# fjetter/distributed

Hardware: AMD Instinct MI355X
Metric: task placements/sec at 1M tasks x 1,024 workers; % of HBM roofline (higher is better)
Workload: dtype int64+f64

## Files before the change

distributed_amd/csrc/dgp_stream.h:

```cpp

#include "dgp_svcmsg.h"

#ifndef DGP_ST_NS
#define DGP_ST_NS st
#endif

#ifndef DGP_STREAM_SHARED_DEFINED
#define DGP_STREAM_SHARED_DEFINED
#define DGP_ST_PRIMARY 1
namespace dgp {
constexpr size_t ST_LDS_BYTES = 22608;
__shared__ __attribute__((aligned(16))) char st_lds_raw[ST_LDS_BYTES];
extern __shared__ __attribute__((aligned(16))) char st_smem[];
}
#else
#undef DGP_ST_PRIMARY
#define DGP_ST_PRIMARY 0
#endif

namespace dgp {
namespace DGP_ST_NS {

__constant__ Dev c_dev;

#ifndef DGP_PHASE_PROBES
#define DGP_PHASE_PROBES 0
#endif
#ifndef DGP_EXE_PRIO
#define DGP_EXE_PRIO 1
#endif
#ifndef DGP_EXE_SLEEP
#define DGP_EXE_SLEEP 1
#endif
#ifndef DGP_EXE_PF
#define DGP_EXE_PF 1
#endif
#ifndef DGP_PROF_GLOBAL
#define DGP_PROF_GLOBAL 0
#endif
#ifndef DGP_REG_PROBES
#define DGP_REG_PROBES 0
#endif
#ifndef DGP_BULK_RESTR
#define DGP_BULK_RESTR 1
#endif
#ifndef DGP_RUN_PAR
#define DGP_RUN_PAR 1
#endif
#ifndef DGP_RB
#define DGP_RB 8
#endif
#ifndef DGP_SCTA
#define DGP_SCTA 1024
#endif
constexpr int SCTA = DGP_SCTA;
#ifndef DGP_WIN
#define DGP_WIN 32
#endif
constexpr int WIN = DGP_WIN;
using SMask = unsigned long long;
static_assert(WIN >= 32 && WIN <= 64, "DGP_WIN must be in [32, 64]");
#ifndef DGP_WAITC
#define DGP_WAITC 1
#endif
constexpr bool WAITC = DGP_WAITC != 0;
constexpr int WAITC_AHEAD = 32;
static_assert(!WAITC || WIN == 32, "DGP_WAITC keeps the candidate-only registrations in the masks' high half");
__host__ __device__ constexpr unsigned long long slot_bits(int s) {
  return WAITC ? ((1ull << s) | (1ull << (s + 32))) : (1ull << s);
}
#ifndef DGP_RS
#define DGP_RS 128
#endif
constexpr int RS = DGP_RS;
constexpr int NE = 64;
#ifndef DGP_DR
#define DGP_DR 512
#endif
constexpr int DR = DGP_DR;
constexpr int PLC = 64;
constexpr int KT_MAX = 24;
constexpr int KX_MAX = 8;
constexpr int RC_MAX = 8;
constexpr int PD = 8;
constexpr int PX = 32;
constexpr int TMAX = 32;
constexpr int NLW = 12;
constexpr int NXW = 52;
constexpr int PG = 64;
constexpr int BIG = 1 << 24;
constexpr int T_CAND = 0x8000;
constexpr int T_W = 0x7fff;
constexpr uint32_t NL_OVF = 0xffffffffu;
static_assert(NLW == SNLW && NXW == SNXW && NL_OVF == SNL_OVF, "dgp_device.h's one-lane needs_what ops use this layout");
constexpr int N_ROLE = 5;
constexpr int E_HDR = 7;
static_assert((DR & (DR - 1)) == 0 && DR >= 64 && DR >= WIN, "DGP_DR must be a power of two >= 64");
static_assert((RS & (RS - 1)) == 0 && RS >= WIN && RS <= DR, "DGP_RS must be a power of two in [WIN, DR]");

enum : uint32_t { F_GLOBAL = 1, F_SELFREL = 2, F_EXACT = 4, F_TOUCHALL = 8, F_BADTOUCH = 16, F_SIMPLE = 32, F_RUNM = 64 };
enum : int { K_COMPLETE = 1, K_PLACE = 2, K_COMPLETE_LR = 3 };
enum : int { SERR_NONE = 0, SERR_PREFIX = 11, SERR_WATCHDOG = 12, SERR_QUEUE = 13, SERR_NEEDS = 14,
             SERR_REC = 15, SERR_CAND = 16, SERR_STAGE = 17, SERR_RANGE = 18, SERR_INV = 19 };

#if DGP_ST_PRIMARY
struct Pos {
  long long seq, bld, pre, reg;
  long long rec_len, walk;
  long long runid_upto;
  long long round_end;
  long long round_start_saved;
  long long prev_placed;
};

struct SRec {
  int32_t w;
  int16_t p;
  int8_t kind;
  int8_t pad;
  int32_t nproc;
  int32_t task;
  int64_t dnet;
  double occ;
  double dur;
};
#else
using st::Pos;
using st::SRec;
#endif

struct SCtl {
  int stop, error, err_task;
  int inv_ok;
  int q_anon;
  int q_prefix;
  int capmax;
  int global_pending;
// ... 339 lines not shown
      sl[PD - 1] = 0u;
      ord -= 1u << 24;
    }
  }
  const bool lj = lane_id() == j;
  d.c.x = lj ? sl[0] : d.c.x;
  d.c.y = lj ? sl[1] : d.c.y;
  d.c.z = lj ? sl[2] : d.c.z;
  d.c.w = lj ? sl[3] : d.c.w;
  d.c1.x = lj ? sl[4] : d.c1.x;
  d.c1.y = lj ? sl[5] : d.c1.y;
  d.c1.z = lj ? sl[6] : d.c1.z;
  d.c1.w = lj ? sl[7] : d.c1.w;
  d.ord = lj ? ord : d.ord;
  return ok;
}

using DTab = const __attribute__((address_space(3))) double*;

__device__ __forceinline__ double resolve_dur(const Dev& D, double d, int p) {
  return d < 0 ? (D.pmaxexec[p] > 0 ? 2 * D.pmaxexec[p] : D.unknown_duration) : d;
}

__device__ __forceinline__ double occ_dict(const WDict& d, int64_t netocc, DTab dt, const Dev& D) {
  const uint32_t n = wd_n(d.ord);
  double res = 0.0;
#pragma unroll
  for (int i = 0; i < PD; i++) {
    if (!ballot((uint32_t)i < n)) break;
    const uint32_t v = wd_slot(d, i);
    const int p = (int)(v >> 24) & (PX - 1);
    const double dv = dt[p];
    const double term = resolve_dur(D, dv, p) * (double)(v & 0xffffffu);
    if ((uint32_t)i < n) res += term;
  }
  return res + (double)netocc / (double)D.bandwidth;
}

__device__ __forceinline__ double occ_dict_r(const WDict& d, double net_bw, DTab dt, const Dev& D) {
  const uint32_t n = wd_n(d.ord);
  double res = 0.0;
  {
    const uint32_t v0 = d.c.x, v1 = d.c.y;
    const double dv0 = dt[(v0 >> 24) & (PX - 1)], dv1 = dt[(v1 >> 24) & (PX - 1)];
    const double t0 = (dv0 < 0 ? D.unknown_duration : dv0) * (double)(v0 & 0xffffffu);
    const double t1 = (dv1 < 0 ? D.unknown_duration : dv1) * (double)(v1 & 0xffffffu);
    if (n > 0u) res += t0;
    if (n > 1u) res += t1;
  }
#pragma unroll
  for (int i = 2; i < PD; i++) {
    if (!ballot((uint32_t)i < n)) break;
    const uint32_t v = wd_slot(d, i);
    const double dv = dt[(v >> 24) & (PX - 1)];
    const double term = (dv < 0 ? D.unknown_duration : dv) * (double)(v & 0xffffffu);
    if ((uint32_t)i < n) res += term;
  }
  return res + net_bw;
}
__device__ __forceinline__ double net_bw_of(int64_t netocc, const Dev& D) {
  return (double)netocc / (double)D.bandwidth;
}

template <bool LW>
__device__ __forceinline__ WDict dict_load(const WPtr<LW>& P, int c) {
  using U4 = typename WPtr<LW>::template P<const Q4>;
  WDict d;
  d.c = ld4(ascast<U4>(P.pcnt + (size_t)c * PD));
  d.c1 = ld4(ascast<U4>(P.pcnt + (size_t)c * PD + 4));
  d.ord = P.plen[c];
  return d;
}

template <bool LW>
__device__ __forceinline__ double occ_of(const WPtr<LW>& P, const Dev& D, int c, DTab dt) {
  return occ_dict(dict_load<LW>(P, c), P.netocc[c], dt, D);
}


__device__ __attribute__((always_inline)) void serr(SCtl& S, int code, int task) {
  if (atomicCAS(&S.error, 0, code) == 0) S.err_task = task;
  vstore(&S.stop, 1);
}


constexpr unsigned long long WATCHDOG = 1600000000ull;
__device__ __forceinline__ unsigned long long rclk() { return __builtin_amdgcn_s_memrealtime(); }
__device__ __forceinline__ bool stalled_for(unsigned long long since, unsigned long long now) {
  return now - since > WATCHDOG;
}

__device__ __forceinline__ int64_t nbv(const Dev& D, int64_t v) { return v >= 0 ? v : D.default_data_size; }
__device__ __forceinline__ bool restr_has(const Dev& D, int x, int w) {
  const RRow rr = restr_row(D, x);
  int64_t lo = rr.r0, hi = rr.r1;
  while (lo < hi) {
    const int64_t mid = (lo + hi) >> 1;
    if (rr.idx[mid] < w) lo = mid + 1;
    else hi = mid;
  }
  return lo < rr.r1 && rr.idx[lo] == w;
}

struct WState {
  int n;
  int pf;
  long long cnt;
  double netocc;
  double wd;
  long long n_idle, n_sat;
};
static_assert(PG == 64 && PX <= 64, "one lane per global dict entry / per prefix");

__device__ __forceinline__ int64_t rl_i64(int64_t v, int l) { return mk64(rlu(lo32(v), l), rlu(hi32(v), l)); }
__device__ __forceinline__ double rl_f64(double v, int l) { return mkd(rlu(dlo(v), l), rlu(dhi(v), l)); }

__device__ __forceinline__ void ws_load(const SCtl& S, WState& g) {
  const int lane = lane_id();
  g.n = S.g_plen;
  g.pf = S.g_pfx[lane];
  g.cnt = S.g_pcnt[lane];
  g.netocc = S.g_netocc;
  g.wd = S.wdur[lane & (PX - 1)];
  g.n_idle = S.n_idle;
  g.n_sat = S.n_sat;
}
__device__ __forceinline__ void ws_store(SCtl& S, const WState& g) {
  const int lane = lane_id();
  if (lane == 0) {
    S.g_plen = g.n;
    S.g_netocc = g.netocc;
    S.n_idle = g.n_idle;
    S.n_sat = g.n_sat;
  }
  S.g_pfx[lane] = g.pf;
  S.g_pcnt[lane] = g.cnt;
  if (lane < PX) S.wdur[lane] = g.wd;
}
__device__ __forceinline__ bool gdict_add(WState& g, int p, int delta) {
  const int lane = lane_id();
  const unsigned long long m = ballot(lane < g.n && g.pf == p);
  if (delta > 0) {
    if (m) {
      if (lane == __builtin_ctzll(m)) g.cnt++;
      return true;
    }
    if (g.n >= PG) return false;
    if (lane == g.n) {
      g.pf = p;
      g.cnt = 1;
    }
    g.n++;
    return true;
  }
  if (!m) return true;
  const int at = __builtin_ctzll(m);
  const long long v = rl_i64(g.cnt, at) - 1;
  if (v > 0) {
    if (lane == at) g.cnt = v;
    return true;
  }
  const int pn = __shfl_down(g.pf, 1);
  const long long cn = __shfl_down(g.cnt, 1);
  if (lane >= at) {
    g.pf = pn;
    g.cnt = cn;
// ... 1239 lines not shown
  if (m) {
    const int ml = __builtin_ctzll(m);
    const uint32_t v = rlu(nl, ml) - 1;
    const bool gone = (v & 0xffu) == 0;
    if (lane == ml) nl = gone ? 0u : v;
    if (gone && lane == NLW - 1) nl -= 0x100u;
    return gone ? nb : 0;
  }
  const int ext = (int)(ctl >> 8) - line_used(nl);
  if (ext > 0) {
    uint32_t* X = D.gw_needs_ext + (size_t)c * NXW;
    const uint32_t xe = lane < NXW ? __hip_atomic_load(X + lane, __ATOMIC_RELAXED, __HIP_MEMORY_SCOPE_AGENT) : 0u;
    const unsigned long long mx = ballot(lane < NXW && xe != 0 && (xe >> 8) == (uint32_t)d);
    if (mx) {
      const int ml = __builtin_ctzll(mx);
      const uint32_t v = rlu(xe, ml) - 1;
      const bool gone = (v & 0xffu) == 0;
      if (lane == ml) __hip_atomic_store(X + ml, gone ? 0u : v, __ATOMIC_RELAXED, __HIP_MEMORY_SCOPE_AGENT);
      if (gone && lane == NLW - 1) nl -= 0x100u;
      __threadfence_block();
      return gone ? nb : 0;
    }
  }
  if (D.evf & EVF_MULTI) return 0;
  serr(S, SERR_NEEDS, d);
  return 0;
}

__device__ __attribute__((always_inline)) int64_t needs_inc(const Dev& D, SCtl& S, int c, uint32_t& nl, int d, int64_t nb, int except) {
  const int lane = lane_id();
  const uint32_t ctl = rlu(nl, NLW - 1);
  if (ctl == NL_OVF) return st_needed_elsewhere(D, d, c, except) ? 0 : nb;
  const unsigned long long m = ballot(lane < NLW - 1 && nl != 0 && (nl >> 8) == (uint32_t)d);
  if (m) {
    const int ml = __builtin_ctzll(m);
    if ((rlu(nl, ml) & 0xffu) == 0xffu) {
      serr(S, SERR_NEEDS, d);
      return 0;
    }
    if (lane == ml) nl += 1;
    return 0;
  }
  const int used = line_used(nl);
  const int ext = (int)(ctl >> 8) - used;
  uint32_t* X = D.gw_needs_ext + (size_t)c * NXW;
  uint32_t xe = 0;
  if (ext > 0) {
    xe = lane < NXW ? __hip_atomic_load(X + lane, __ATOMIC_RELAXED, __HIP_MEMORY_SCOPE_AGENT) : 0u;
    const unsigned long long mx = ballot(lane < NXW && xe != 0 && (xe >> 8) == (uint32_t)d);
    if (mx) {
      const int ml = __builtin_ctzll(mx);
      if ((rlu(xe, ml) & 0xffu) == 0xffu) {
        serr(S, SERR_NEEDS, d);
        return 0;
      }
      if (lane == ml) __hip_atomic_store(X + ml, xe + 1, __ATOMIC_RELAXED, __HIP_MEMORY_SCOPE_AGENT);
      __threadfence_block();
      return 0;
    }
  }
  const unsigned long long em = ballot(lane < NLW - 1 && nl == 0);
  if (em) {
    if (lane == __builtin_ctzll(em)) nl = ((uint32_t)d << 8) | 1u;
    if (lane == NLW - 1) nl += 0x100u;
    return nb;
  }
  if (ext < NXW) {
    const unsigned long long ex = ballot(lane < NXW && xe == 0);
    const int ml = __builtin_ctzll(ex);
    if (lane == ml) __hip_atomic_store(X + ml, ((uint32_t)d << 8) | 1u, __ATOMIC_RELAXED, __HIP_MEMORY_SCOPE_AGENT);
    if (lane == NLW - 1) nl = nl + 0x100u;
    __threadfence_block();
    return nb;
  }
  if (lane == NLW - 1) nl = NL_OVF;
  return nb;
}

__device__ __forceinline__ unsigned long long lm_eq(unsigned a, unsigned b) { return __builtin_amdgcn_uicmp(a, b, 32); }
__device__ __forceinline__ unsigned long long lm_ne(unsigned a, unsigned b) { return __builtin_amdgcn_uicmp(a, b, 33); }
__device__ __forceinline__ bool lm_has(unsigned long long m) { return (m >> lane_id()) & 1ull; }
constexpr unsigned long long NL_LINE = (1ull << (NLW - 1)) - 1;

__device__ __forceinline__ bool needs_dec_all(const uint4& E, int L0, int k, int c, uint32_t& nl, int64_t& freed) {
  const uint32_t ctl = rlu(nl, NLW - 1);
  const unsigned long long used = lm_ne(nl, 0u) & NL_LINE;
  if (ctl == NL_OVF || (int)(ctl >> 8) != __builtin_popcountll(used)) return false;
  const uint32_t key = nl >> 8;
  const unsigned long long one = lm_eq(nl & 0xffu, 1u) & used;
  unsigned long long hit = 0;
  int64_t fr = 0;
  int ngone = 0;
  for (int i = 0; i < k; i++) {
    if (rl((int)E.y, L0 + i) == c) continue;
    const unsigned long long m = lm_eq(key, rlu(E.x, L0 + i)) & used;
    if (!m) return false;
    hit |= m;
    if (m & one) {
      fr += mk64(rlu(E.z, L0 + i), rlu(E.w, L0 + i));
      ngone++;
    }
  }
  if (hit) nl = lm_has(hit & one) ? 0u : (lm_has(hit) ? nl - 1u : nl);
  if (ngone) nl = lane_id() == NLW - 1 ? nl - ((uint32_t)ngone << 8) : nl;
  freed = fr;
  return true;
}

__device__ __forceinline__ bool needs_inc_all(const uint4& E, int L0, int k, int c, uint32_t& nl, int64_t& added) {
  const uint32_t ctl = rlu(nl, NLW - 1);
  const unsigned long long used = lm_ne(nl, 0u) & NL_LINE;
  if (ctl == NL_OVF || (int)(ctl >> 8) != __builtin_popcountll(used)) return false;
  const uint32_t key = nl >> 8;
  const unsigned long long full = lm_eq(nl & 0xffu, 0xffu) & used;
  unsigned long long freem = ~used & NL_LINE;
  unsigned long long hit = 0;
  uint32_t nn = nl;
  int64_t ad = 0;
  int nins = 0;
  for (int i = 0; i < k; i++) {
    if (rl((int)E.y, L0 + i) == c) continue;
    const uint32_t d = rlu(E.x, L0 + i);
    const unsigned long long m = lm_eq(key, d) & used;
    if (m) {
      if (m & full) return false;
      hit |= m;
    } else {
      if (!freem) return false;
      const int l = __builtin_ctzll(freem);
      freem &= freem - 1;
      nn = lane_id() == l ? (d << 8) | 1u : nn;
      ad += mk64(rlu(E.z, L0 + i), rlu(E.w, L0 + i));
      nins++;
    }
  }
  if (hit) nn = lm_has(hit) ? nn + 1u : nn;
  if (nins) nn = lane_id() == NLW - 1 ? nn + ((uint32_t)nins << 8) : nn;
  nl = nn;
  added = ad;
  return true;
}

__device__ __attribute__((always_inline)) void needs_reset(const Dev& D, int c, uint32_t& nl) {
  const int lane = lane_id();
  const uint32_t ctl = rlu(nl, NLW - 1);
  if (ctl == NL_OVF || (ctl >> 8) != 0) {
    if (lane < NXW) __hip_atomic_store(D.gw_needs_ext + (size_t)c * NXW + lane, 0u, __ATOMIC_RELAXED, __HIP_MEMORY_SCOPE_AGENT);
    __threadfence_block();
  }
  if (lane < NLW) nl = 0;
}

struct Out {
  int nrec, npl;
  size_t st0;
  __device__ void rec(const Dev& D, int kind, int w, int p, int64_t dnet, double occ, int np, int task, double dur) {
    if (lane_id() == 0 && nrec < PLC) {
      SRec rc;
      rc.w = w;
      rc.p = (int16_t)p;
      rc.kind = (int8_t)kind;
      rc.pad = 0;
      rc.nproc = np;
      rc.task = task;
      rc.dnet = dnet;
      rc.occ = occ;
      rc.dur = dur;
      D.srec[st0 + nrec] = rc;
    }
    nrec++;
  }
  __device__ void place(const Dev& D, int task, int w, int64_t comm, double start, int64_t wsnb, int route) {
    if (lane_id() == 0 && npl < PLC) {
      D.s2_task[st0 + npl] = task;
      D.s2_worker[st0 + npl] = w;
      D.s2_comm[st0 + npl] = comm;
      D.s2_start[st0 + npl] = start;
      D.s2_wsnb[st0 + npl] = wsnb;
      D.s2_route[st0 + npl] = (int8_t)route;
    }
    npl++;
  }
};

template <bool LW>
__device__ __forceinline__ bool dict_update(const WPtr<LW>& P, int c, int p, int delta, WDict& d) {
  using U4 = typename WPtr<LW>::template P<Q4>;
  d = dict_load<LW>(P, c);
  const bool ok = dict_add(d, p, delta);
  if (lane_id() == 0) {
    st4(ascast<U4>(P.pcnt + (size_t)c * PD), d.c);
    st4(ascast<U4>(P.pcnt + (size_t)c * PD + 4), d.c1);
    P.plen[c] = d.ord;
  }
  return ok;
}

__device__ __forceinline__ int release_succ(SLds& L, SMask old, int from = -1) {
  const SMask succ = WAITC ? (old & 0xffffffffull) : old;
  if (!succ) return -1;
  int bs = __builtin_ctzll(succ);
  long long best = vload(&L.sid[bs]);
  for (SMask m = succ & (succ - 1); m; m &= m - 1) {
    const int b = __builtin_ctzll(m);
    const long long v = vload(&L.sid[b]);
    if (v < best) {
      best = v;
      bs = b;
    }
  }
  if (WAITC && ((old >> 32) >> bs) & 1ull) {
    const int pc = __hip_atomic_fetch_add(&L.predc[bs], -1, __ATOMIC_RELAXED, __HIP_MEMORY_SCOPE_WORKGROUP);
    if (TR3 && pc == 1) {
      const Dev& D = c_dev;
      TR(L.sid[bs], 20);
      if (from >= 0) trace_at(D, L.sid[bs], 21, (unsigned long long)L.sid[from]);
    }
    return -1;
// ... 1 lines not shown
  if (atomicSub(&L.pred[bs], 1) == 1) {
    atomicOr(&L.c.ready, 1ull << bs);
    if (TRL) {
      const Dev& D = c_dev;
      TR(L.sid[bs], 1);
      if (TR3 && from >= 0) trace_at(D, L.sid[bs], 19, (unsigned long long)L.sid[from]);
    }
    return bs;
  }
  return -1;
}
template <bool LW>
__device__ __forceinline__ int release_worker(SLds& L, const WPtr<LW>& P, int s, int c) {
  const SMask bit = slot_bits(s);
  return release_succ(L, __hip_atomic_fetch_and(&P.mask[c], ~bit, __ATOMIC_RELAXED, __HIP_MEMORY_SCOPE_WORKGROUP) & ~bit,
                      DGP_TRACE ? s : -1);
}

template <bool LW>
__device__ __attribute__((always_inline)) void release_slot(const Dev& D, SLds& L, const WPtr<LW>& P, int s, bool all) {
  const int lane = lane_id();
  const SMask bit = slot_bits(s);
  auto rel = [&](int c) {
    release_succ(L, __hip_atomic_fetch_and(&P.mask[c], ~bit, __ATOMIC_RELAXED, __HIP_MEMORY_SCOPE_WORKGROUP) & ~bit,
                 DGP_TRACE ? s : -1);
  };
  if (all) {
    for (int c = lane; c < D.W; c += 64) rel(c);
  } else {
    const int nt = L.ntouch[s];
    if (lane < nt) rel((int)L.touch[s][lane] & T_W);
  }
}

template <class O>
__device__ __attribute__((always_inline)) void finish_slot(const Dev& D, SLds& L, int s, long long r, const O& o, int npops, bool direct) {
  const int lane = lane_id();
  const int q = (int)(r & (RS - 1));
  if (lane == 0) {
    RMeta me;
    me.npl = o.npl;
    me.nrec = (uint8_t)(direct ? 0 : o.nrec);
    me.npops = (uint8_t)npops;
    me.direct = direct ? 1 : 0;
    me.pad = 0;
    L.rmeta[q] = me;
  }
  __threadfence_block();
  if (lane == 0) {
    vstore(&L.rdone[q], r + 1);
    atomicOr(&L.c.freem, 1ull << s);
  }
  if (DGP_TRACE && lane == 0) TR(r, 5);
}

__device__ __forceinline__ unsigned wmin_u32(unsigned v) {
  v = min(v, (unsigned)__builtin_amdgcn_update_dpp((int)v, (int)v, 0xb1, 0xf, 0xf, false));
  v = min(v, (unsigned)__builtin_amdgcn_update_dpp((int)v, (int)v, 0x4e, 0xf, 0xf, false));
  v = min(v, (unsigned)__builtin_amdgcn_update_dpp((int)v, (int)v, 0x141, 0xf, 0xf, false));
  v = min(v, (unsigned)__builtin_amdgcn_update_dpp((int)v, (int)v, 0x140, 0xf, 0xf, false));
  return min(min(rlu(v, 0), rlu(v, 16)), min(rlu(v, 32), rlu(v, 48)));
}

struct Key {
  double start;
  int64_t nb;
  int w;
  int64_t comm;
};
__device__ __forceinline__ bool key_less(const Key& a, const Key& b) {
  if (a.start != b.start) return a.start < b.start;
  if (a.nb != b.nb) return a.nb < b.nb;
  return a.w < b.w;
}

__device__ __forceinline__ uint64_t start_key(double x) {
  const uint64_t b = x == 0.0 ? 0ull : (uint64_t)__double_as_longlong(x);
  return (b >> 63) ? ~b : (b | (1ull << 63));
}
__device__ __forceinline__ uint64_t rl64(uint64_t v, int l) {
  return ((uint64_t)rlu((unsigned)(v >> 32), l) << 32) | rlu((unsigned)v, l);
}

__device__ __forceinline__ DTab stim_durations(const Dev& D, SLds& L, const uint4& E, long long r) {
  const int lane = lane_id();
  const auto t = (__attribute__((address_space(3))) double*)(double*)L.dur[threadIdx.x >> 6];
  if (D.P <= PD) {
    if (lane >= 3 && lane < 7) {
      t[2 * (lane - 3)] = mkd(E.x, E.y);
      t[2 * (lane - 3) + 1] = mkd(E.z, E.w);
    }
  } else if (lane < D.P) {
    t[lane] = D.dring[(size_t)(r & (DR - 1)) * PX + lane];
  }
  return (DTab)(const double*)t;
}

template <bool LW>
__device__ __attribute__((always_inline)) bool exe_local(const Dev& D, SLds& L, const WPtr<LW>& P, int s, long long r, int qmode, bool exact, const uint4& E,
                                                         int& woke) {
  SCtl& S = L.c;
  const int lane = lane_id();
  const DTab durv = stim_durations(D, L, E, r);
  const int t = rl((int)E.x, 0), w = rl((int)E.y, 0), p = rl((int)E.z, 0);
  const uint32_t flags = rlu(E.w, 0);
  const int64_t nbt = mk64(rlu(E.x, 1), rlu(E.y, 1));
  const unsigned cnts = rlu(E.z, 1);
  const int kt = cnts & 0xff, nrel = (cnts >> 8) & 0xff, nf = (cnts >> 16) & 0xff;
  const double dobs = mkd(rlu(E.x, 2), rlu(E.y, 2));
  const int TD = E_HDR, RL0 = E_HDR + kt, FX0 = RL0 + nrel;
#if DGP_PHASE_PROBES
  unsigned long long tph = mclk();
  auto phase = [&](int k) {
    const unsigned long long n = mclk();
    PROF(if (lane == 0) atomicAdd(&S.prof[k], n - tph));
    tph = n;
  };
#else
  auto phase = [](int) {};
#endif
  const int tot_new = rl((int)E.w, 2);
  if (!exact) {
    const int ntch = L.ntouch[s];
    bool bad = false;
    if (lane < ntch) {
      const int tv0 = L.touch[s][lane];
      const int c = tv0 & T_W;
      const uint32_t ctl = P.needs[(size_t)c * NLW + NLW - 1];
      const int slack = (WAITC && lane > 0 && (tv0 & T_CAND)) ? NXW / 2 : 0;
      bad = ctl == NL_OVF || (int)(ctl >> 8) + tot_new + slack > NLW - 1 + NXW;
    }
    if (ballot(bad)) return false;
  }
  Out o;
  o.nrec = 0;
  o.npl = 0;
  o.st0 = (size_t)(r & (RS - 1)) * PLC;
  phase(11);
  if (DGP_TRACE == 2 && lane == 0) TR(r, 0);
  if (TR3 && lane == 0) TR(r, 8);
  const int nt = L.ntouch[s];
  const bool tl = lane < nt;
  const int tv = tl ? (int)L.touch[s][lane] : 0;
  const int cj = tv & T_W;
  const bool candl = (tv & T_CAND) != 0;
  const bool wc = WAITC && tl && lane > 0 && candl;
  int np = 0, nth = 1;
  WDict dj;
  dj.c = make_uint4(0, 0, 0, 0);
  dj.c1 = make_uint4(0, 0, 0, 0);
  dj.ord = 0;
  int64_t net = 0, nbj = 0;
  if (tl) nth = P.nthreads[cj];
  if (tl && !wc) {
    np = P.nproc[cj];
    dj = dict_load<LW>(P, cj);
    net = P.netocc[cj];
    nbj = P.nbytes[cj];
  }
  const int capw = P.cap[w];
  uint32_t nl = line_load<LW>(P, w);
  const unsigned long long wm = ballot(tl && cj == w);
  if (!wm) {
    serr(S, SERR_INV, 700000000 + (int)r);
    return true;
  }
  const int jw = __builtin_ctzll(wm);
  const bool isw = lane == jw;
  const bool nth1 = !ballot(tl && nth != 1);
  phase(16);
  if (DGP_TRACE == 2 && lane == 0) TR(r, 1);
  if (TR3 && lane == 0) {
    TR(r, 9);
    trace_at(D, r, 22, (unsigned long long)(nf | kt << 8 | nrel << 16 | nt << 24));
    trace_at(D, r, 23, (unsigned long long)vload(&L.predc[s]));
  }
  int64_t dnet = 0;
  int64_t freed = 0;
  if (needs_dec_all(E, TD, kt, w, nl, freed)) dnet = -freed;
  else for (int i = 0; i < kt; i++) {
    const int L_ = TD + i;
    const int h = rl((int)E.y, L_);
    if (h == w) continue;
    const int d = rl((int)E.x, L_);
    const int64_t nb = mk64(rlu(E.z, L_), rlu(E.w, L_));
    dnet -= needs_dec(D, S, w, nl, d, nb, t);
  }
  if (TR4 && lane == 0) TR(r, 24);
  const int npw = rl(np, jw) - 1;
  if (npw == 0) needs_reset(D, w, nl);
  line_store<LW>(P, w, nl);
  if (TR4 && lane == 0) TR(r, 25);
  if (isw) {
    dict_add(dj, p, -1);
    np = npw;
    net += dnet;
  }
  if (TR4 && lane == 0) TR(r, 26);
  double nbw = net_bw_of(net, D);
  phase(17);
  if (DGP_TRACE == 2 && lane == 0) TR(r, 3);
  if (TR3 && lane == 0) TR(r, 10);
  double occj = occ_dict_r(dj, nbw, durv, D);
  double stkj = nth1 ? occj : occj / (double)nth;
  o.rec(D, K_COMPLETE, w, p, dnet, mkd(rlu(dlo(occj), jw), rlu(dhi(occj), jw)), npw, t, dobs);
  if (isw) nbj += (flags & F_SELFREL) ? 0 : nbt;
  for (int i = 0; i < nrel; i++) {
    const int h = rl((int)E.x, RL0 + i);
    const int64_t nb = mk64(rlu(E.z, RL0 + i), rlu(E.w, RL0 + i));
    if (tl && !wc && cj == h) nbj -= nb;
  }
  bool released = false;
  {
    const bool ro = tl && !isw && !candl;
    if (ballot(ro)) {
      if (ro) P.nbytes[cj] = nbj;
      __builtin_amdgcn_s_waitcnt(0xc07f);
      __atomic_signal_fence(__ATOMIC_SEQ_CST);
      if (ro) release_worker<LW>(L, P, s, cj);
      released = ro;
    }
  }
  if (TR3 && lane == 0) TR(r, 11);
  if (WAITC && ballot(wc)) {
    if (vload(&L.predc[s]) != 0) {
      if (DGP_EXE_PRIO) __builtin_amdgcn_s_setprio(1);
      while (vload(&L.predc[s]) != 0) __builtin_amdgcn_s_sleep(1);
      if (DGP_EXE_PRIO) __builtin_amdgcn_s_setprio(3);
    }
    lds_fence();
    if (wc) {
      np = P.nproc[cj];
      dj = dict_load<LW>(P, cj);
      net = P.netocc[cj];
      nbj = P.nbytes[cj];
    }
    for (int i = 0; i < nrel; i++) {
      const int h = rl((int)E.x, RL0 + i);
      const int64_t nb = mk64(rlu(E.z, RL0 + i), rlu(E.w, RL0 + i));
      if (wc && cj == h) nbj -= nb;
    }
    if (wc) {
      nbw = net_bw_of(net, D);
      occj = occ_dict_r(dj, nbw, durv, D);
      stkj = nth1 ? occj : occj / (double)nth;
    }
    if (!exact) {
      bool bad = false;
      if (wc) {
        const uint32_t ctl = P.needs[(size_t)cj * NLW + NLW - 1];
        bad = ctl == NL_OVF || (int)(ctl >> 8) + tot_new > NLW - 1 + NXW;
      }
      if (ballot(bad)) {
        while (vload(&S.seq_pos) != r) __builtin_amdgcn_s_sleep(1);
        lds_fence();
        exact = true;
      }
    }
  }
  phase(12);
  if (DGP_TRACE == 2 && lane == 0) TR(r, 4);
  if (TR3 && lane == 0) TR(r, 12);
  int off = FX0;
  for (int j = 0; j < nf; j++) {
    const int x = rl((int)E.x, off), px = rl((int)E.y, off);
    const int hz = rl((int)E.z, off);
    const int kx = hz & 0xff, nc = (hz >> 8) & 0xff;
    int64_t comm = 0;
    bool cand = false;
    for (int i = 0; i < kx; i++) {
      const int L2 = off + 1 + i;
      const int hi = rl((int)E.y, L2);
      const int64_t nbi = mk64(rlu(E.z, L2), rlu(E.w, L2));
      if (cj == hi) cand = true;
      else comm += nbi;
    }
    if (hz & (1 << 16)) {
      cand = false;
      for (int i = 0; i < nc; i++) cand = cand || cj == rl((int)E.x, off + 1 + kx + i);
    }
    cand = cand && tl;
    Key k;
    k.start = stkj + (double)comm / (double)D.bandwidth;
    k.nb = nbj;
    k.w = cj;
    k.comm = comm;
    phase(18);
    if (TR3 && lane == 0 && j == 0) TR(r, 13);
    const unsigned long long cm = ballot(cand);
    if (!cm) {
      serr(S, SERR_CAND, x);
      return true;
    }
    int jb = __builtin_ctzll(cm);
    Key best;
    double bs = mkd(rlu(dlo(k.start), jb), rlu(dhi(k.start), jb));
    for (unsigned long long rm = cm & (cm - 1); rm; rm &= rm - 1) {
      const int jq = __builtin_ctzll(rm);
      const double qs = mkd(rlu(dlo(k.start), jq), rlu(dhi(k.start), jq));
      bool less = qs < bs;
      if (!(qs != bs)) {
        const int64_t qn = mk64(rlu(lo32(k.nb), jq), rlu(hi32(k.nb), jq));
        const int64_t bn = mk64(rlu(lo32(k.nb), jb), rlu(hi32(k.nb), jb));
        less = qn != bn ? qn < bn : rl(k.w, jq) < rl(k.w, jb);
      }
      if (less) {
        bs = qs;
        jb = jq;
      }
    }
    best.start = bs;
    best.nb = mk64(rlu(lo32(k.nb), jb), rlu(hi32(k.nb), jb));
    best.w = rl(k.w, jb);
    best.comm = mk64(rlu(lo32(k.comm), jb), rlu(hi32(k.comm), jb));
    if (TR4 && lane == 0 && j == 0) TR(r, 27);
    const int cb = best.w;
    if (j == nf - 1 && nt > 2) {
      const bool early = tl && !isw && lane != jb && !released;
      if (ballot(early)) {
        if (early) {
          using U4 = typename WPtr<LW>::template P<Q4>;
          P.nproc[cj] = np;
          st4(ascast<U4>(P.pcnt + (size_t)cj * PD), dj.c);
          st4(ascast<U4>(P.pcnt + (size_t)cj * PD + 4), dj.c1);
          P.plen[cj] = dj.ord;
          P.netocc[cj] = net;
          P.nbytes[cj] = nbj;
        }
        __builtin_amdgcn_s_waitcnt(0xc07f);
        __atomic_signal_fence(__ATOMIC_SEQ_CST);
        if (early) release_worker<LW>(L, P, s, cj);
        released = released || early;
        if (TRL && lane == 0) TR(r, 3);
      }
    }
    phase(19);
    if (TR3 && lane == 0 && j == 0) TR(r, 14);
    o.place(D, x, cb, best.comm, best.start, best.nb, ROUTE_NONROOTISH);
    uint32_t nlc = line_load<LW>(P, cb);
    if (TR4 && lane == 0 && j == 0) TR(r, 28);
    if (exact) {
      if (lane == 0) D.proc_on[rl((int)E.x, 0)] = -1;
      __threadfence_block();
    }
    int64_t dn = 0;
    if (!needs_inc_all(E, off + 1, kx, cb, nlc, dn)) for (int i = 0; i < kx; i++) {
      const int L2 = off + 1 + i;
      if (rl((int)E.y, L2) == cb) continue;
      const int d = rl((int)E.x, L2);
      const int64_t nb = mk64(rlu(E.z, L2), rlu(E.w, L2));
      dn += needs_inc(D, S, cb, nlc, d, nb, x);
    }
    if (TR4 && lane == 0 && j == 0) TR(r, 29);
    line_store<LW>(P, cb, nlc);
    const bool isb = lane == jb;
    bool okp = true;
    if (isb) {
      okp = dict_add(dj, px, +1);
      np += 1;
      net += dn;
    }
    if (TR4 && lane == 0 && j == 0) TR(r, 30);
    if (dn != 0) nbw = isb ? net_bw_of(net, D) : nbw;
    if (ballot(!okp)) serr(S, SERR_PREFIX, x);
    if (TR4 && lane == 0 && j == 0) TR(r, 31);
    if (exact && lane == 0) {
      D.proc_on[x] = cb;
      D.state[x] = S_PROCESSING;
    }
    occj = occ_dict_r(dj, nbw, durv, D);
    stkj = nth1 ? occj : occj / (double)nth;
    o.rec(D, K_PLACE, cb, px, dn, mkd(rlu(dlo(occj), jb), rlu(dhi(occj), jb)), rl(np, jb), x, 0.0);
    off += 1 + kx + nc;
    phase(20);
    if (TR3 && lane == 0 && j == 0) TR(r, 15);
  }
  if (DGP_TRACE == 2 && lane == 0) TR(r, 6);
  if (TR3 && lane == 0) TR(r, 16);
  if (tl && !isw && !released) {
    using U4 = typename WPtr<LW>::template P<Q4>;
    P.nproc[cj] = np;
    st4(ascast<U4>(P.pcnt + (size_t)cj * PD), dj.c);
    st4(ascast<U4>(P.pcnt + (size_t)cj * PD + 4), dj.c1);
    P.plen[cj] = dj.ord;
    P.netocc[cj] = net;
    P.nbytes[cj] = nbj;
  }
  if (nt > 1) {
    __builtin_amdgcn_s_waitcnt(0xc07f);
    __atomic_signal_fence(__ATOMIC_SEQ_CST);
    if (tl && !isw && !released) release_worker<LW>(L, P, s, cj);
  }
  if (TRL && lane == 0) TR(r, 4);
  int pops = 0;
  if (qmode != 0 && !D.sat_inf) {
    const int slots = capw - rl(np, jw);
    if (slots > capw || o.npl + slots > PLC - 1) {
      serr(S, SERR_INV, 600000000 + (int)r);
      return true;
    }
    if (slots > 0) {
      pops = slots;
      if (qmode == 3) pops = (int)min((long long)slots, vload(&S.qlen));
    }
    const int qp = S.q_prefix;
    for (int i = 0; i < pops; i++) {
      const double st = stkj + 0.0;
      o.place(D, -1, w, 0, mkd(rlu(dlo(st), jw), rlu(dhi(st), jw)), mk64(rlu(lo32(nbj), jw), rlu(hi32(nbj), jw)),
              ROUTE_ROOTISH_Q);
      bool okq = true;
      if (isw) {
        okq = dict_add(dj, qp, +1);
        np += 1;
      }
      if (ballot(!okq)) serr(S, SERR_PREFIX, -1);
      occj = occ_dict_r(dj, nbw, durv, D);
      stkj = nth1 ? occj : occj / (double)nth;
      o.rec(D, K_PLACE, w, qp, 0, mkd(rlu(dlo(occj), jw), rlu(dhi(occj), jw)), rl(np, jw), -1, 0.0);
    }
  }
  if (TR3 && lane == 0) TR(r, 17);
  if (isw) {
    using U4 = typename WPtr<LW>::template P<Q4>;
    P.nproc[cj] = np;
    st4(ascast<U4>(P.pcnt + (size_t)cj * PD), dj.c);
    st4(ascast<U4>(P.pcnt + (size_t)cj * PD + 4), dj.c1);
    P.plen[cj] = dj.ord;
    P.netocc[cj] = net;
    P.nbytes[cj] = nbj;
  }
  __builtin_amdgcn_s_waitcnt(0xc07f);
  __atomic_signal_fence(__ATOMIC_SEQ_CST);
  int wk = -1;
  if (lane == jw) wk = release_worker<LW>(L, P, s, w);
  if (TR3 && lane == 0) TR(r, 18);
  woke = rl(wk, jw);
  phase(13);
  phase(21);
  phase(14);
  finish_slot(D, L, s, r, o, pops, false);
  phase(15);
  return true;
}

template <bool LW>
__device__ __attribute__((always_inline)) bool exe_run(const Dev& D, SLds& L, const WPtr<LW>& P, int s, long long r,
                                                       const uint4& E) {
  SCtl& S = L.c;
  const int lane = lane_id();
  if (L.ntouch[s] != 1) return false;
  const int w = rl((int)E.y, 0);
  const bool sl = lane < WIN && lane != s;
  const long long offl = sl ? vload(&L.sid[lane]) - r : -1;
  const bool el = sl && offl >= 1 && offl < 64 && vload(&L.pred[lane]) == 1 && vload(&L.ntouch[lane]) == 1 &&
                  (L.touch[lane][0] & T_W) == w && (vload(&L.flags[lane]) & (F_GLOBAL | F_EXACT | F_SIMPLE)) == F_SIMPLE;
  int my_slot = lane == 0 ? s : -1;
  int n = 1;
  while (n < 64) {
    const unsigned long long m = ballot(el && offl == n);
    if (!m) break;
    if (lane == n) my_slot = __builtin_ctzll(m);
    n++;
  }
  uint4 h0 = make_uint4(0, 0, 0, 0), h1 = h0, h2 = h0, ed = h0, er = h0, dq[4];
  bool ok = false, needs_m = false;
  if (lane < n) {
    const uint4* row = D.desc + (size_t)((r + lane) & (DR - 1)) * NE;
    h0 = row[0];
    h1 = row[1];
    h2 = row[2];
#pragma unroll
    for (int q = 0; q < 4; q++) dq[q] = row[3 + q];
    ed = row[E_HDR];
    er = row[E_HDR + 1];
  }
  {
    bool same = true;
#pragma unroll
    for (int q = 0; q < 4; q++)
      same = same && dq[q].x == rlu(E.x, 3 + q) && dq[q].y == rlu(E.y, 3 + q) && dq[q].z == rlu(E.z, 3 + q) &&
             dq[q].w == rlu(E.w, 3 + q);
    const int kt = h1.z & 0xff, nrel = (h1.z >> 8) & 0xff, nf = (h1.z >> 16) & 0xff;
    const uint4 erel = kt == 0 ? ed : er;
    ok = lane < n && (int)h0.y == w && !(h0.w & F_GLOBAL) && nf == 0 && kt <= 1 && nrel <= 1 &&
         (nrel == 0 || (int)erel.x == w) && same;
    er = erel;
    needs_m = ok && kt == 1 && (int)ed.y != w;
  }
  const unsigned long long nm = ballot(needs_m);
  const uint32_t nl = line_load<LW>(P, w);
  const uint32_t ctl = rlu(nl, NLW - 1);
  if (ctl == NL_OVF) return false;
  unsigned long long cut = ballot(!ok);
  int d_ml = -1;
  if (nm) {
    const uint32_t d0 = rlu(ed.x, __builtin_ctzll(nm));
    cut |= ballot(needs_m && ed.x != d0);
    const unsigned long long em = ballot(lane < NLW - 1 && nl != 0 && (nl >> 8) == d0);
    if (!em) {
      cut |= nm & (0ull - nm);
// ... 1493 lines not shown
```

Baseline: 1.060 million.

## Outline cold paths and streamline needs-line scans in exe_local hot loop

Moves rare paths (error reporting, per-dep needs fallback, wide duration rows, exact-mode bookkeeping, oldest-wait) into noinline cold functions and marks branches with expectations, aiming to shrink the inlined hot kernel and its register pressure. The dependency scans in needs_inc_all/needs_dec_all become branchless with a partially unrolled loop. Candidate entries are rotated once with ds_bpermute so dependency lanes start at lane 0, and the released-bytes loop is computed once and reused. The added risks are call overhead and ABI register spills on the cold paths, plus four extra bpermutes on every placement.

New measurement: 1.190 million, median of 6. 1.12x the previous value.

```diff
diff --git a/distributed_amd/csrc/dgp_stream.h b/distributed_amd/csrc/dgp_stream.h
--- a/distributed_amd/csrc/dgp_stream.h
+++ b/distributed_amd/csrc/dgp_stream.h
@@ -53,6 +53,7 @@
 #ifndef DGP_SCTA
 #define DGP_SCTA 1024
 #endif
+#define DGP_COLD __attribute__((noinline, cold))
 constexpr int SCTA = DGP_SCTA;
 #ifndef DGP_WIN
 #define DGP_WIN 32
@@ -558,6 +559,7 @@
   if (atomicCAS(&S.error, 0, code) == 0) S.err_task = task;
   vstore(&S.stop, 1);
 }
+__device__ DGP_COLD void serr_cold(int code, int task) { serr(st_L().c, code, task); }
 
 
 constexpr unsigned long long WATCHDOG = 1600000000ull;
@@ -1963,58 +1965,89 @@
 __device__ __forceinline__ bool lm_has(unsigned long long m) { return (m >> lane_id()) & 1ull; }
 constexpr unsigned long long NL_LINE = (1ull << (NLW - 1)) - 1;
 
+template <class F>
+__device__ __forceinline__ void each_dep(int k, F&& f) {
+#pragma unroll
+  for (int i = 0; i < 4; i++)
+    if (i < k) f(i);
+  for (int i = 4; i < k; i++) f(i);
+}
+
+struct NeedsLine {
+  uint32_t key;
+  unsigned long long used;
+  bool ok;
+};
+__device__ __forceinline__ NeedsLine needs_line(uint32_t nl) {
+  const uint32_t ctl = rlu(nl, NLW - 1);
+  NeedsLine n;
+  n.used = lm_ne(nl, 0u) & NL_LINE;
+  n.ok = ctl != NL_OVF && (int)(ctl >> 8) == __builtin_popcountll(n.used);
+  n.key = nl >> 8;
+  return n;
+}
+
 __device__ __forceinline__ bool needs_dec_all(const uint4& E, int L0, int k, int c, uint32_t& nl, int64_t& freed) {
-  const uint32_t ctl = rlu(nl, NLW - 1);
-  const unsigned long long used = lm_ne(nl, 0u) & NL_LINE;
-  if (ctl == NL_OVF || (int)(ctl >> 8) != __builtin_popcountll(used)) return false;
-  const uint32_t key = nl >> 8;
-  const unsigned long long one = lm_eq(nl & 0xffu, 1u) & used;
+  const NeedsLine n = needs_line(nl);
+  if (!n.ok) return false;
+  const unsigned long long one = lm_eq(nl & 0xffu, 1u) & n.used;
   unsigned long long hit = 0;
   int64_t fr = 0;
   int ngone = 0;
-  for (int i = 0; i < k; i++) {
-    if (rl((int)E.y, L0 + i) == c) continue;
-    const unsigned long long m = lm_eq(key, rlu(E.x, L0 + i)) & used;
-    if (!m) return false;
+  bool miss = false;
+  each_dep(k, [&](int i) {
+    const int l = L0 + i;
+    if (rl((int)E.y, l) == c) return;
+    const unsigned long long m = lm_eq(n.key, rlu(E.x, l)) & n.used;
+    miss = miss || !m;
     hit |= m;
     if (m & one) {
-      fr += mk64(rlu(E.z, L0 + i), rlu(E.w, L0 + i));
+      fr += mk64(rlu(E.z, l), rlu(E.w, l));
       ngone++;
     }
-  }
+  });
+  if (miss) return false;
   if (hit) nl = lm_has(hit & one) ? 0u : (lm_has(hit) ? nl - 1u : nl);
   if (ngone) nl = lane_id() == NLW - 1 ? nl - ((uint32_t)ngone << 8) : nl;
   freed = fr;
   return true;
 }
 
+__device__ __forceinline__ uint4 entries_from(const uint4& E, int first) {
+  const int a = ((lane_id() + first) & 63) << 2;
+  return make_uint4((unsigned)__builtin_amdgcn_ds_bpermute(a, (int)E.x), (unsigned)__builtin_amdgcn_ds_bpermute(a, (int)E.y),
+                    (unsigned)__builtin_amdgcn_ds_bpermute(a, (int)E.z), (unsigned)__builtin_amdgcn_ds_bpermute(a, (int)E.w));
+}
+
 __device__ __forceinline__ bool needs_inc_all(const uint4& E, int L0, int k, int c, uint32_t& nl, int64_t& added) {
-  const uint32_t ctl = rlu(nl, NLW - 1);
-  const unsigned long long used = lm_ne(nl, 0u) & NL_LINE;
-  if (ctl == NL_OVF || (int)(ctl >> 8) != __builtin_popcountll(used)) return false;
-  const uint32_t key = nl >> 8;
-  const unsigned long long full = lm_eq(nl & 0xffu, 0xffu) & used;
-  unsigned long long freem = ~used & NL_LINE;
+  const NeedsLine n = needs_line(nl);
+  if (!n.ok) return false;
+  const unsigned long long full = lm_eq(nl & 0xffu, 0xffu) & n.used;
+  unsigned long long freem = ~n.used & NL_LINE;
   unsigned long long hit = 0;
   uint32_t nn = nl;
   int64_t ad = 0;
   int nins = 0;
-  for (int i = 0; i < k; i++) {
-    if (rl((int)E.y, L0 + i) == c) continue;
-    const uint32_t d = rlu(E.x, L0 + i);
-    const unsigned long long m = lm_eq(key, d) & used;
+  bool bad = false;
+  each_dep(k, [&](int i) {
+    const int l = L0 + i;
+    if (rl((int)E.y, l) == c) return;
+    const uint32_t d = rlu(E.x, l);
+    const unsigned long long m = lm_eq(n.key, d) & n.used;
     if (m) {
-      if (m & full) return false;
+      bad = bad || (m & full);
       hit |= m;
+    } else if (!freem) {
+      bad = true;
     } else {
-      if (!freem) return false;
-      const int l = __builtin_ctzll(freem);
+      const int f = __builtin_ctzll(freem);
       freem &= freem - 1;
-      nn = lane_id() == l ? (d << 8) | 1u : nn;
-      ad += mk64(rlu(E.z, L0 + i), rlu(E.w, L0 + i));
+      nn = lane_id() == f ? (d << 8) | 1u : nn;
+      ad += mk64(rlu(E.z, l), rlu(E.w, l));
       nins++;
     }
-  }
+  });
+  if (bad) return false;
   if (hit) nn = lm_has(hit) ? nn + 1u : nn;
   if (nins) nn = lane_id() == NLW - 1 ? nn + ((uint32_t)nins << 8) : nn;
   nl = nn;
@@ -2182,6 +2215,12 @@
   return ((uint64_t)rlu((unsigned)(v >> 32), l) << 32) | rlu((unsigned)v, l);
 }
 
+__device__ DGP_COLD void dur_row_cold(long long r) {
+  const Dev& D = c_dev;
+  const int lane = lane_id();
+  const auto t = (__attribute__((address_space(3))) double*)(double*)st_L().dur[threadIdx.x >> 6];
+  if (lane < D.P) t[lane] = D.dring[(size_t)(r & (DR - 1)) * PX + lane];
+}
 __device__ __forceinline__ DTab stim_durations(const Dev& D, SLds& L, const uint4& E, long long r) {
   const int lane = lane_id();
   const auto t = (__attribute__((address_space(3))) double*)(double*)L.dur[threadIdx.x >> 6];
@@ -2190,11 +2229,62 @@
       t[2 * (lane - 3)] = mkd(E.x, E.y);
       t[2 * (lane - 3) + 1] = mkd(E.z, E.w);
     }
-  } else if (lane < D.P) {
-    t[lane] = D.dring[(size_t)(r & (DR - 1)) * PX + lane];
+  } else {
+    dur_row_cold(r);
   }
   return (DTab)(const double*)t;
 }
+
+struct NeedsRes {
+  uint32_t nl;
+  int64_t v;
+};
+__device__ DGP_COLD NeedsRes needs_dec_each(uint4 E, int L0, int k, int c, uint32_t nl, int t) {
+  const Dev& D = c_dev;
+  SCtl& S = st_L().c;
+  int64_t v = 0;
+  for (int i = 0; i < k; i++) {
+    const int L_ = L0 + i;
+    if (rl((int)E.y, L_) == c) continue;
+    v += needs_dec(D, S, c, nl, rl((int)E.x, L_), mk64(rlu(E.z, L_), rlu(E.w, L_)), t);
+  }
+  return NeedsRes{nl, v};
+}
+__device__ DGP_COLD NeedsRes needs_inc_each(uint4 E, int L0, int k, int c, uint32_t nl, int x) {
+  const Dev& D = c_dev;
+  SCtl& S = st_L().c;
+  int64_t v = 0;
+  for (int i = 0; i < k; i++) {
+    const int L2 = L0 + i;
+    if (rl((int)E.y, L2) == c) continue;
+    v += needs_inc(D, S, c, nl, rl((int)E.x, L2), mk64(rlu(E.z, L2), rlu(E.w, L2)), x);
+  }
+  return NeedsRes{nl, v};
+}
+__device__ DGP_COLD bool restr_cand_cold(unsigned ex, int L0, int nc, int cj) {
+  bool cand = false;
+  for (int i = 0; i < nc; i++) cand = cand || cj == rl((int)ex, L0 + i);
+  return cand;
+}
+__device__ DGP_COLD double stack_time_cold(double occ, int nth) { return occ / (double)nth; }
+__device__ DGP_COLD void exact_left_cold(int t) {
+  if (lane_id() == 0) c_dev.proc_on[t] = -1;
+  __threadfence_block();
+}
+__device__ DGP_COLD void exact_placed_cold(int x, int cb) {
+  if (lane_id() == 0) {
+    c_dev.proc_on[x] = cb;
+    c_dev.state[x] = S_PROCESSING;
+  }
+}
+__device__ DGP_COLD void wait_oldest_cold(long long r) {
+  SCtl& S = st_L().c;
+  while (vload(&S.seq_pos) != r) __builtin_amdgcn_s_sleep(1);
+  lds_fence();
+}
+
+#define LIKELY(x) __builtin_expect(!!(x), 1)
+#define UNLIKELY(x) __builtin_expect(!!(x), 0)
 
 template <bool LW>
 __device__ __attribute__((always_inline)) bool exe_local(const Dev& D, SLds& L, const WPtr<LW>& P, int s, long long r, int qmode, bool exact, const uint4& E,
@@ -2230,7 +2320,7 @@
       const int slack = (WAITC && lane > 0 && (tv0 & T_CAND)) ? NXW / 2 : 0;
       bad = ctl == NL_OVF || (int)(ctl >> 8) + tot_new + slack > NLW - 1 + NXW;
     }
-    if (ballot(bad)) return false;
+    if (UNLIKELY(ballot(bad))) return false;
   }
   Out o;
   o.nrec = 0;
@@ -2261,8 +2351,8 @@
   const int capw = P.cap[w];
   uint32_t nl = line_load<LW>(P, w);
   const unsigned long long wm = ballot(tl && cj == w);
-  if (!wm) {
-    serr(S, SERR_INV, 700000000 + (int)r);
+  if (UNLIKELY(!wm)) {
+    serr_cold(SERR_INV, 700000000 + (int)r);
     return true;
   }
   const int jw = __builtin_ctzll(wm);
@@ -2277,14 +2367,11 @@
   }
   int64_t dnet = 0;
   int64_t freed = 0;
-  if (needs_dec_all(E, TD, kt, w, nl, freed)) dnet = -freed;
-  else for (int i = 0; i < kt; i++) {
-    const int L_ = TD + i;
-    const int h = rl((int)E.y, L_);
-    if (h == w) continue;
-    const int d = rl((int)E.x, L_);
-    const int64_t nb = mk64(rlu(E.z, L_), rlu(E.w, L_));
-    dnet -= needs_dec(D, S, w, nl, d, nb, t);
+  if (LIKELY(needs_dec_all(E, TD, kt, w, nl, freed))) dnet = -freed;
+  else {
+    const NeedsRes nr = needs_dec_each(E, TD, kt, w, nl, t);
+    nl = nr.nl;
+    dnet = -nr.v;
   }
   if (TR4 && lane == 0) TR(r, 24);
   const int npw = rl(np, jw) - 1;
@@ -2302,14 +2389,16 @@
   if (DGP_TRACE == 2 && lane == 0) TR(r, 3);
   if (TR3 && lane == 0) TR(r, 10);
   double occj = occ_dict_r(dj, nbw, durv, D);
-  double stkj = nth1 ? occj : occj / (double)nth;
+  double stkj = LIKELY(nth1) ? occj : stack_time_cold(occj, nth);
   o.rec(D, K_COMPLETE, w, p, dnet, mkd(rlu(dlo(occj), jw), rlu(dhi(occj), jw)), npw, t, dobs);
   if (isw) nbj += (flags & F_SELFREL) ? 0 : nbt;
+  int64_t relj = 0;
   for (int i = 0; i < nrel; i++) {
     const int h = rl((int)E.x, RL0 + i);
     const int64_t nb = mk64(rlu(E.z, RL0 + i), rlu(E.w, RL0 + i));
-    if (tl && !wc && cj == h) nbj -= nb;
-  }
+    if (cj == h) relj += nb;
+  }
+  if (tl && !wc) nbj -= relj;
   bool released = false;
   {
     const bool ro = tl && !isw && !candl;
@@ -2335,15 +2424,11 @@
       net = P.netocc[cj];
       nbj = P.nbytes[cj];
     }
-    for (int i = 0; i < nrel; i++) {
-      const int h = rl((int)E.x, RL0 + i);
-      const int64_t nb = mk64(rlu(E.z, RL0 + i), rlu(E.w, RL0 + i));
-      if (wc && cj == h) nbj -= nb;
-    }
+    if (wc) nbj -= relj;
     if (wc) {
       nbw = net_bw_of(net, D);
       occj = occ_dict_r(dj, nbw, durv, D);
-      stkj = nth1 ? occj : occj / (double)nth;
+      stkj = LIKELY(nth1) ? occj : stack_time_cold(occj, nth);
     }
     if (!exact) {
       bool bad = false;
@@ -2351,9 +2436,8 @@
         const uint32_t ctl = P.needs[(size_t)cj * NLW + NLW - 1];
         bad = ctl == NL_OVF || (int)(ctl >> 8) + tot_new > NLW - 1 + NXW;
       }
-      if (ballot(bad)) {
-        while (vload(&S.seq_pos) != r) __builtin_amdgcn_s_sleep(1);
-        lds_fence();
+      if (UNLIKELY(ballot(bad))) {
+        wait_oldest_cold(r);
         exact = true;
       }
     }
@@ -2368,16 +2452,15 @@
     const int kx = hz & 0xff, nc = (hz >> 8) & 0xff;
     int64_t comm = 0;
     bool cand = false;
-    for (int i = 0; i < kx; i++) {
-      const int L2 = off + 1 + i;
-      const int hi = rl((int)E.y, L2);
-      const int64_t nbi = mk64(rlu(E.z, L2), rlu(E.w, L2));
+    const uint4 F = entries_from(E, off + 1);
+    each_dep(kx, [&](int i) {
+      const int hi = rl((int)F.y, i);
+      const int64_t nbi = mk64(rlu(F.z, i), rlu(F.w, i));
       if (cj == hi) cand = true;
       else comm += nbi;
-    }
-    if (hz & (1 << 16)) {
-      cand = false;
-      for (int i = 0; i < nc; i++) cand = cand || cj == rl((int)E.x, off + 1 + kx + i);
+    });
+    if (UNLIKELY(hz & (1 << 16))) {
+      cand = restr_cand_cold(E.x, off + 1 + kx, nc, cj);
     }
     cand = cand && tl;
     Key k;
@@ -2388,8 +2471,8 @@
     phase(18);
     if (TR3 && lane == 0 && j == 0) TR(r, 13);
     const unsigned long long cm = ballot(cand);
-    if (!cm) {
-      serr(S, SERR_CAND, x);
+    if (UNLIKELY(!cm)) {
+      serr_cold(SERR_CAND, x);
       return true;
     }
     int jb = __builtin_ctzll(cm);
@@ -2439,17 +2522,14 @@
     o.place(D, x, cb, best.comm, best.start, best.nb, ROUTE_NONROOTISH);
     uint32_t nlc = line_load<LW>(P, cb);
     if (TR4 && lane == 0 && j == 0) TR(r, 28);
-    if (exact) {
-      if (lane == 0) D.proc_on[rl((int)E.x, 0)] = -1;
-      __threadfence_block();
+    if (UNLIKELY(exact)) {
+      exact_left_cold(t);
     }
     int64_t dn = 0;
-    if (!needs_inc_all(E, off + 1, kx, cb, nlc, dn)) for (int i = 0; i < kx; i++) {
-      const int L2 = off + 1 + i;
-      if (rl((int)E.y, L2) == cb) continue;
-      const int d = rl((int)E.x, L2);
-      const int64_t nb = mk64(rlu(E.z, L2), rlu(E.w, L2));
-      dn += needs_inc(D, S, cb, nlc, d, nb, x);
+    if (UNLIKELY(!needs_inc_all(F, 0, kx, cb, nlc, dn))) {
+      const NeedsRes nr = needs_inc_each(E, off + 1, kx, cb, nlc, x);
+      nlc = nr.nl;
+      dn = nr.v;
     }
     if (TR4 && lane == 0 && j == 0) TR(r, 29);
     line_store<LW>(P, cb, nlc);
@@ -2462,14 +2542,11 @@
     }
     if (TR4 && lane == 0 && j == 0) TR(r, 30);
     if (dn != 0) nbw = isb ? net_bw_of(net, D) : nbw;
-    if (ballot(!okp)) serr(S, SERR_PREFIX, x);
+    if (UNLIKELY(ballot(!okp))) serr_cold(SERR_PREFIX, x);
     if (TR4 && lane == 0 && j == 0) TR(r, 31);
-    if (exact && lane == 0) {
-      D.proc_on[x] = cb;
-      D.state[x] = S_PROCESSING;
-    }
+    if (UNLIKELY(exact)) exact_placed_cold(x, cb);
     occj = occ_dict_r(dj, nbw, durv, D);
-    stkj = nth1 ? occj : occj / (double)nth;
+    stkj = LIKELY(nth1) ? occj : stack_time_cold(occj, nth);
     o.rec(D, K_PLACE, cb, px, dn, mkd(rlu(dlo(occj), jb), rlu(dhi(occj), jb)), rl(np, jb), x, 0.0);
     off += 1 + kx + nc;
     phase(20);
@@ -2495,8 +2572,8 @@
   int pops = 0;
   if (qmode != 0 && !D.sat_inf) {
     const int slots = capw - rl(np, jw);
-    if (slots > capw || o.npl + slots > PLC - 1) {
-      serr(S, SERR_INV, 600000000 + (int)r);
+    if (UNLIKELY(slots > capw || o.npl + slots > PLC - 1)) {
+      serr_cold(SERR_INV, 600000000 + (int)r);
       return true;
     }
     if (slots > 0) {
@@ -2513,9 +2590,9 @@
         okq = dict_add(dj, qp, +1);
         np += 1;
       }
-      if (ballot(!okq)) serr(S, SERR_PREFIX, -1);
+      if (UNLIKELY(ballot(!okq))) serr_cold(SERR_PREFIX, -1);
       occj = occ_dict_r(dj, nbw, durv, D);
-      stkj = nth1 ? occj : occj / (double)nth;
+      stkj = LIKELY(nth1) ? occj : stack_time_cold(occj, nth);
       o.rec(D, K_PLACE, w, qp, 0, mkd(rlu(dlo(occj), jw), rlu(dhi(occj), jw)), rl(np, jw), -1, 0.0);
     }
   }
```
